# MariBax/self-supervised-depth-estimation

Hardware: AMD Instinct MI355X
Metric: training images/sec at 192x640 bs12 (resnet18 depth+pose, 4-scale photometric+smoothness) (higher is better)
Workload: dtype f32 (1x1 convolutions: bf16x3 split operands, fp32 accumulate); 1 GPU; BASELINE configs[1]: resnet18 depth+pose, 192x640, per-GPU batch 12, 4 scales, frames {0,-1,+1}, automasking, Adam lr 1e-4; random-init weights; global_batch=12, parallelism=dp1, tiebreak_noise=on-device counter RNG, setup_steps=0, step_launch=eager (one launch per kernel)

## Files before the change

include/depthcore.h:

```cpp
#ifndef DEPTHCORE_H
#define DEPTHCORE_H

#include <stddef.h>
#include <stdint.h>

#ifdef __cplusplus
extern "C" {
#endif

#define DC_OK 0
#define DC_EINVAL (-1)
#define DC_ELAUNCH (-2)
#define DC_EWORKSPACE (-3)
#define DC_EEMPTY (-4)

#define DC_MAX_SCALES 4

#define DC_OPT_NO_AUTOMASK 1u
#define DC_OPT_AVG_REPROJ 2u
#define DC_OPT_NO_SSIM 4u
#define DC_OPT_ALIGN_CORNERS 8u
#define DC_OPT_PRED_MASK 32u
#define DC_OPT_PHOTO_SPLIT 64u
#define DC_OPT_PHOTO_FULL 128u
// ... 150 lines not shown
int dc_bn_stats(const float* x, float* part, int N, int C, int HW, int groups, void* stream);
int dc_bn_finalize(const float* part, int nparts, int ppg, double count, const float* gamma, const float* beta,
                   float* running_mean, float* running_var, float* mean, float* invstd, float* scale, float* shift,
                   int C, int groups, float eps, float momentum, void* stream);
int dc_bn_apply(const float* x, const float* res, const float* scale, const float* shift, float* y, void* relu_mask,
                int N, int C, int HW, int relu, int groups, void* stream);
int dc_bn_bwd_finalize(const float* part, int nparts, int ppg, double count, const float* gamma, const float* mean,
                       const float* invstd, float* coef, float* dgamma, float* dbeta, int C, int groups, void* stream);
int dc_bn_bwd_apply(const float* x, const float* gp, const float* coef, float* dx, int N, int C, int HW, int groups,
                    void* stream);

int dc_bn_eval_coef(const float* gamma, const float* beta, const float* running_mean, const float* running_var, float* scale,
                    float* shift, float* invstd, int C, float eps, void* stream);
size_t dc_bn_eval_bwd_workspace(int N, int C, int HW);
int dc_bn_eval_bwd(const float* x, const float* y, const float* gy, const float* scale, const float* running_mean,
                   const float* invstd, float* dx, float* dres, float* dgamma, float* dbeta, void* ws, int N, int C, int HW,
                   int relu, void* stream);

int dc_maxpool3x3s2_fwd(const float* x, float* y, uint8_t* code, int NC, int H, int W, void* stream);
int dc_maxpool3x3s2_bwd(const float* gy, const uint8_t* code, float* dx, int NC, int H, int W, void* stream);
int dc_maxpool3x3s2_bwd_add(const float* gy, const uint8_t* code, float* dx, const float* addend, int NC, int H, int W,
                            void* stream);

size_t dc_wino3x3_workspace(int B, int Ci, int Co, int H, int W);
int dc_wino3x3_fwd(const float* x, const float* weight, float* y, void* ws, int B, int Ci, int Co, int H, int W,
                   void* stream);
int dc_wino3x3_dgrad(const float* gy, const float* weight, float* gx, void* ws, int B, int Ci, int Co, int H, int W,
                     void* stream);
int dc_wino3x3_dgrad_add(const float* gy, const float* weight, float* gx, const float* addend, void* ws, int B, int Ci, int Co,
                         int H, int W, void* stream);

int dc_wino3x3_bn_ok(int B, int Ci, int Co, int H, int W, int groups);
int dc_wino3x3_stat_parts(int B, int Ci, int Co, int H, int W, int groups, int* ppg);
int dc_wino3x3_bwd_parts(int B, int Ci, int Co, int H, int W, int groups, int* ppg);
int dc_wino3x3_fwd_bn(const float* x, const float* weight, float* y, void* ws, int B, int Ci, int Co, int H, int W,
                      const dc_bn_fold* bn, void* stream);
int dc_wino3x3_dgrad_bn(const float* gy, const float* weight, float* gx, const float* addend, void* ws, int B, int Ci, int Co,
                        int H, int W, const dc_bn_fold* bn, void* stream);
int dc_wino3x3_wgrad_bn(const float* x, const float* gy, float* dweight, void* ws, int B, int Ci, int Co, int H, int W,
                        const dc_bn_fold* bn, void* stream);

int dc_conv_profile_enable(int max_launches, int every);
int dc_conv_profile_collect(int kind, double* ms, double* algorithmic_flops, double* executed_flops,
                            double* algorithmic_bytes, int* launches);

size_t dc_wino3x3_wgrad_workspace(int B, int Ci, int Co, int H, int W);
// ... 175 lines not shown
```

self-supervised-depth-estimation_amd/csrc/bn.hip:

```cpp
#include "dc_common.h"

namespace dc {

constexpr int BN_CHUNK = 4096;

__device__ __forceinline__ float block_sum256(float v, float* sm) {
    v = wave_sum(v);
    __syncthreads();
    if ((threadIdx.x & 63) == 0) sm[threadIdx.x >> 6] = v;
    __syncthreads();
    return (sm[0] + sm[1]) + (sm[2] + sm[3]);
}

constexpr int BN_U = 4;
struct BnItems {
    int wave, lane, ipp, nitems, lo, hi, ns, HW;
    __device__ __forceinline__ BnItems(int ns_, int HW_, int lo_, int hi_) : lo(lo_), hi(hi_), ns(ns_), HW(HW_) {
        wave = __builtin_amdgcn_readfirstlane(threadIdx.x >> 6); lane = threadIdx.x & 63;
        if (ns > 1) { ipp = (HW + 255) >> 8; nitems = ((ns - wave + 3) >> 2) * ipp; }
        else { ipp = 1; nitems = (hi - lo + 1023) >> 10; }
    }
    __device__ __forceinline__ bool at(int k, int& nn, int& i) const {
        bool ok;
        if (ns > 1) {
// ... 128 lines not shown
        const size_t base = ((size_t)n * C + c) * HW;
        for (int i = lo + threadIdx.x; i < hi; i += 256) {
            float v = fmaf(x[base + i], a, b);
            if (res) v += res[base + i];
            y[base + i] = relu ? fmaxf(v, 0.f) : v;
        }
    }
}

__device__ __forceinline__ float4 bn_apply_bits(float4 g, unsigned bits) {
    g.x = (bits & 1u) ? g.x : 0.f; g.y = (bits & 2u) ? g.y : 0.f; g.z = (bits & 4u) ? g.z : 0.f; g.w = (bits & 8u) ? g.w : 0.f;
    return g;
}
struct BnMaskWords { unsigned long long w[4]; };
__device__ __forceinline__ unsigned bn_bits_of(const BnMaskWords& m) {
    const int l = threadIdx.x & 63;
    return (unsigned)((m.w[0] >> l) & 1ull) | ((unsigned)((m.w[1] >> l) & 1ull) << 1) | ((unsigned)((m.w[2] >> l) & 1ull) << 2) |
           ((unsigned)((m.w[3] >> l) & 1ull) << 3);
}
__device__ __forceinline__ unsigned bn_bits_of(float4 yv) {
    return (yv.x > 0.f ? 1u : 0u) | (yv.y > 0.f ? 2u : 0u) | (yv.z > 0.f ? 4u : 0u) | (yv.w > 0.f ? 8u : 0u);
}

template <int MODE>
__global__ __launch_bounds__(256) void bn_bwd_stats_kernel(const float* __restrict__ x, const float* __restrict__ y, const float* __restrict__ gy,
                                                           const float* __restrict__ mean, const float* __restrict__ invstd, float* __restrict__ part, int C,
                                                           int HW, int n_per_group, const unsigned long long* __restrict__ mask, int ns) {
    __shared__ float sm[8];
    const int c = blockIdx.y, n0 = blockIdx.z * ns;
    const int gc = (n0 / n_per_group) * C + c;
    const float m = mean[gc], is = invstd[gc];
    const int lo = blockIdx.x * BN_CHUNK, hi = min(lo + BN_CHUNK, HW);
    float s = 0.f, q = 0.f;
    if ((HW & 3) == 0) {
        const BnItems it(ns, HW, lo, hi);
        for (int k0 = 0; k0 < it.nitems; k0 += BN_U) {
            float4 xv[BN_U], g[BN_U], yv[BN_U];
            BnMaskWords mw[BN_U];
            bool ok[BN_U];
#pragma unroll
            for (int u = 0; u < BN_U; ++u) {
                int nn, i;
                ok[u] = it.at(k0 + u, nn, i);
                const size_t plane = (size_t)(n0 + nn) * C + c, off = plane * HW + i;
                xv[u] = *reinterpret_cast<const float4*>(x + off);
                g[u] = *reinterpret_cast<const float4*>(gy + off);
                if (MODE == 1) mw[u] = *reinterpret_cast<const BnMaskWords*>(mask + (plane * ((HW + 255) >> 8) + (i >> 8)) * 4);
                if (MODE == 2) yv[u] = *reinterpret_cast<const float4*>(y + off);
            }
#pragma unroll
            for (int u = 0; u < BN_U; ++u) {
                float4 gg = g[u];
                if (MODE == 1) gg = bn_apply_bits(gg, bn_bits_of(mw[u]));
                if (MODE == 2) gg = bn_apply_bits(gg, bn_bits_of(yv[u]));
                if (!ok[u]) gg = make_float4(0.f, 0.f, 0.f, 0.f);
                s += (gg.x + gg.y) + (gg.z + gg.w);
                q += (gg.x * (xv[u].x - m) + gg.y * (xv[u].y - m)) + (gg.z * (xv[u].z - m) + gg.w * (xv[u].w - m));
            }
        }
    } else {
        const size_t base = ((size_t)n0 * C + c) * HW;
        for (int i = lo + threadIdx.x; i < hi; i += 256) {
            float g = gy[base + i];
            if (MODE != 0 && !(y[base + i] > 0.f)) g = 0.f;
            s += g; q += g * (x[base + i] - m);
        }
    }
    block_sum256x2(s, q, sm);
    q *= is;
    if (threadIdx.x == 0) {
        float* o = part + (((size_t)c * gridDim.z + blockIdx.z) * gridDim.x + blockIdx.x) * 2;
        o[0] = s; o[1] = q;
    }
}

template <int MODE>
__global__ __launch_bounds__(256) void bn_bwd_apply_kernel(const float* __restrict__ x, const float* __restrict__ y, const float* __restrict__ gy,
                                                           const float* __restrict__ mean, const float* __restrict__ invstd, const float* __restrict__ gamma,
                                                           const float* __restrict__ part, float* __restrict__ dgamma, float* __restrict__ dbeta, float* __restrict__ dx,
                                                           float* __restrict__ dres, int C, int HW, int n_per_group,
                                                           int groups, const unsigned long long* __restrict__ mask, int ns) {
    const int c = blockIdx.y, n0 = blockIdx.z * ns, n = n0;
    const int nparts = gridDim.z * gridDim.x, per = nparts / groups;
    const int gidx = n / n_per_group;
    const float count = (float)n_per_group * (float)HW;
    float s, q;
    bn_reduce_partials(part, c, nparts, per, gidx, s, q);
    if (blockIdx.x == 0 && n == 0) {
        float ts = 0.f, tq = 0.f;
        for (int g2 = 0; g2 < groups; ++g2) {
            float s2, q2;
            bn_reduce_partials(part, c, nparts, per, g2, s2, q2);
            ts += s2; tq += q2;
        }
        if (threadIdx.x == 0) {
            if (dbeta) dbeta[c] = ts;
            if (dgamma) dgamma[c] = tq;
        }
    }
    const int gc = gidx * C + c;
    const float m = mean[gc], is = invstd[gc], k = gamma[c] * is, a = s / count, bq = (q / count) * is;
    const int lo = blockIdx.x * BN_CHUNK, hi = min(lo + BN_CHUNK, HW);
    if ((HW & 3) == 0) {
        const BnItems it(ns, HW, lo, hi);
        for (int k0 = 0; k0 < it.nitems; k0 += BN_U) {
            float4 xv[BN_U], g[BN_U], yv[BN_U];
            BnMaskWords mw[BN_U];
            size_t off[BN_U];
            bool ok[BN_U];
#pragma unroll
            for (int u = 0; u < BN_U; ++u) {
                int nn, i;
                ok[u] = it.at(k0 + u, nn, i);
                const size_t plane = (size_t)(n0 + nn) * C + c;
                off[u] = plane * HW + i;
                xv[u] = *reinterpret_cast<const float4*>(x + off[u]);
                g[u] = *reinterpret_cast<const float4*>(gy + off[u]);
                if (MODE == 1) mw[u] = *reinterpret_cast<const BnMaskWords*>(mask + (plane * ((HW + 255) >> 8) + (i >> 8)) * 4);
                if (MODE == 2) yv[u] = *reinterpret_cast<const float4*>(y + off[u]);
            }
#pragma unroll
            for (int u = 0; u < BN_U; ++u) {
                float4 gg = g[u];
                if (MODE == 1) gg = bn_apply_bits(gg, bn_bits_of(mw[u]));
                if (MODE == 2) gg = bn_apply_bits(gg, bn_bits_of(yv[u]));
                float4 d;
                d.x = k * (gg.x - a - (xv[u].x - m) * bq); d.y = k * (gg.y - a - (xv[u].y - m) * bq);
                d.z = k * (gg.z - a - (xv[u].z - m) * bq); d.w = k * (gg.w - a - (xv[u].w - m) * bq);
                if (ok[u]) {
                    if (dres) *reinterpret_cast<float4*>(dres + off[u]) = gg;
                    *reinterpret_cast<float4*>(dx + off[u]) = d;
                }
            }
        }
    } else {
        const size_t base = ((size_t)n * C + c) * HW;
        for (int i = lo + threadIdx.x; i < hi; i += 256) {
            float g = gy[base + i];
            if (MODE != 0 && !(y[base + i] > 0.f)) g = 0.f;
            if (dres) dres[base + i] = g;
            dx[base + i] = k * (g - a - (x[base + i] - m) * bq);
        }
    }
}

}

using namespace dc;
#define ST ((hipStream_t)stream)

static int bn_ns(int n_per_group, int HW) {
    if ((HW & 3) || HW * 2 > BN_CHUNK) return 1;
    int best = 1;
    for (int d = 2; d <= n_per_group; ++d)
        if (n_per_group % d == 0 && d * HW <= BN_CHUNK) best = d;
    return best;
}

extern "C" size_t dc_bn_workspace(int N, int C, int HW) {
    if (N <= 0 || C <= 0 || HW <= 0) return 0;
    return ((size_t)C * N * ceil_div(HW, BN_CHUNK) * 2 + 2 * (size_t)C * N) * sizeof(float);
}
// ... 15 lines not shown
    DC_CHECK_LAUNCH();
    hipLaunchKernelGGL(bn_apply_kernel, dim3(chunks, C, N / ns), dim3(256), 0, ST, x, res, (const float*)part, save_mean,
                       save_invstd, running_mean, running_var, gamma, beta, y, C, HW, relu, N / groups, groups, eps, momentum,
                       (HW & 3) ? (unsigned long long*)nullptr : (unsigned long long*)relu_mask, ns);
    DC_CHECK_LAUNCH();
    return DC_OK;
}

extern "C" int dc_bn_relu_bwd(const float* x, const float* y, const float* gy, const float* gamma,
                              const float* save_mean, const float* save_invstd, float* dx, float* dres, float* dgamma,
                              float* dbeta, void* ws, const void* relu_mask, int N, int C, int HW, int relu, int groups,
                              void* stream) {
    if (!x || !gy || !gamma || !save_mean || !save_invstd || !dx || !ws || N <= 0 || C <= 0 || HW <= 0) return DC_EINVAL;
    const unsigned long long* mk = (HW & 3) ? nullptr : (const unsigned long long*)relu_mask;
    if (relu && !y && !mk) return DC_EINVAL;
    if (groups < 1 || N % groups) return DC_EINVAL;
    const int chunks = ceil_div(HW, BN_CHUNK), ns = bn_ns(N / groups, HW);
    float* part = (float*)ws;
    const dim3 grid(chunks, C, N / ns);
    const int mode = !relu ? 0 : (mk ? 1 : 2);
#define BN_BWD(MODE)                                                                                                             \
    do {                                                                                                                         \
        hipLaunchKernelGGL(bn_bwd_stats_kernel<MODE>, grid, dim3(256), 0, ST, x, y, gy, save_mean, save_invstd, part, C, HW,      \
                           N / groups, mk, ns);                                                                                  \
        DC_CHECK_LAUNCH();                                                                                                       \
        hipLaunchKernelGGL(bn_bwd_apply_kernel<MODE>, grid, dim3(256), 0, ST, x, y, gy, save_mean, save_invstd, gamma,            \
                           (const float*)part, dgamma, dbeta, dx, dres, C, HW, N / groups, groups, mk, ns);                      \
        DC_CHECK_LAUNCH();                                                                                                       \
    } while (0)
    if (mode == 0) BN_BWD(0);
    else if (mode == 1) BN_BWD(1);
    else BN_BWD(2);
#undef BN_BWD
    return DC_OK;
}

namespace dc {

__device__ __forceinline__ void block_sum256x2_all(float& a, float& b, float* sm8) {
    __syncthreads();
    block_sum256x2(a, b, sm8);
}

__global__ __launch_bounds__(256) void bn_finalize_kernel(const float2* __restrict__ part, int nparts, int ppg, float count,
                                                          const float* __restrict__ gamma, const float* __restrict__ beta,
                                                          float* __restrict__ run_mean, float* __restrict__ run_var,
                                                          float* __restrict__ mean, float* __restrict__ invstd,
                                                          float* __restrict__ scale, float* __restrict__ shift, int C, int groups,
                                                          float eps, float momentum) {
    __shared__ float sm[8];
// ... 466 lines not shown
    return dc_maxpool3x3s2_bwd_add(gy, code, dx, nullptr, NC, H, W, stream);
}

extern "C" int dc_maxpool3x3s2_bwd_add(const float* gy, const uint8_t* code, float* dx, const float* addend, int NC, int H, int W,
                                       void* stream) {
    if (!gy || !code || !dx || NC <= 0 || H < 2 || W < 2 || NC > 65535) return DC_EINVAL;
    const int Ho = (H + 2 - 3) / 2 + 1, Wo = (W + 2 - 3) / 2 + 1;
    if (addend && (W & 7)) {
        const int rc = dc_maxpool3x3s2_bwd_add(gy, code, dx, nullptr, NC, H, W, stream);
        return rc != DC_OK ? rc : dc::add_inplace(dx, addend, (size_t)NC * H * W, (hipStream_t)stream);
    }
    if ((W & 7) == 0)
        hipLaunchKernelGGL(dc::maxpool_bwd8_kernel, dim3(dc::ceil_div(H * (W >> 3), 256), NC), dim3(256), 0, (hipStream_t)stream, gy, code,
                           dx, H, W, Ho, Wo, addend);
    else if ((W & 3) == 0)
        hipLaunchKernelGGL(dc::maxpool_bwd_kernel<true>, dim3(dc::ceil_div(H * (W >> 2), 256), NC), dim3(256), 0,
                           (hipStream_t)stream, gy, code, dx, H, W, Ho, Wo);
    else
        hipLaunchKernelGGL(dc::maxpool_bwd_kernel<false>, dim3(dc::ceil_div(H * W, 256), NC), dim3(256), 0,
                           (hipStream_t)stream, gy, code, dx, H, W, Ho, Wo);
    DC_CHECK_LAUNCH();
    return DC_OK;
}
```

self-supervised-depth-estimation_amd/depthcore/_lib.py:

```python
import ctypes
import os
from ctypes import (POINTER, Structure, c_char_p, c_double, c_float, c_int, c_int32, c_size_t, c_uint8, c_uint32,
                    c_uint64, c_void_p)

import torch

_HERE = os.path.dirname(os.path.abspath(__file__))
PRODUCT_LIB = os.path.join(_HERE, "libdepthcore.so")
LIB_PATH = os.environ.get("DEPTHCORE_LIB") or PRODUCT_LIB
IS_VARIANT = os.path.realpath(LIB_PATH) != os.path.realpath(PRODUCT_LIB)
MAX_SCALES = 4

OPT_NO_AUTOMASK = 1
OPT_AVG_REPROJ = 2
OPT_NO_SSIM = 4
OPT_ALIGN_CORNERS = 8
OPT_NO_GRAD = 16
OPT_PRED_MASK = 32
OPT_PHOTO_SPLIT, OPT_PHOTO_FULL = 64, 128
PREC_F32, PREC_BF16 = 0, 1
PASS_FWD, PASS_DGRAD, PASS_WGRAD = 0, 1, 2

_ERR = {-1: "DC_EINVAL (bad shape / null pointer / unsupported option)",
        -2: "DC_ELAUNCH (hip launch failed)",
# ... 113 lines not shown
        "dc_flip_concat": (i, [p, p, i, i, i, i, p]),
        "dc_disp_post_process": (i, [p, p, i, i, i, f, f, p]),
        "dc_depth_png16": (i, [p, p, i, i, i, i, i, f, p]),
        "dc_pose_ate": (i, [p, p, p, i, i, i, p]),
        "dc_disp_render_ws_bytes": (z, [i, i, i, i, i]),
        "dc_disp_render": (i, [p, p, p, p, i, i, i, i, i, c_double, p, z, p]),
        "dc_bn_bwd_finalize": (i, [p, i, i, c_double, p, p, p, p, p, p, i, i, p]),
        "dc_bn_bwd_apply": (i, [p, p, p, p, i, i, i, i, p]),
        "dc_conv1x1_bn_ok": (i, [i, i, i, i, i]),
        "dc_conv1x1_stat_parts": (i, [i, i, i, i, i, i, i, POINTER(c_int)]),
        "dc_conv1x1_bwd_parts": (i, [i, i, i, i, i, i, POINTER(c_int)]),
        "dc_conv1x1_fwd_bn": (i, [p, p, p, i, i, i, i, i, i, POINTER(BnFold), p]),
        "dc_conv1x1_dgrad_bn": (i, [p, p, p, p, i, i, i, i, i, i, POINTER(BnFold), p]),
        "dc_conv1x1_wgrad_bn": (i, [p, p, p, p, i, i, i, i, i, i, POINTER(BnFold), p]),
        "dc_wino3x3_bn_ok": (i, [i, i, i, i, i, i]),
        "dc_wino3x3_stat_parts": (i, [i, i, i, i, i, i, POINTER(c_int)]),
        "dc_wino3x3_bwd_parts": (i, [i, i, i, i, i, i, POINTER(c_int)]),
        "dc_wino3x3_fwd_bn": (i, [p, p, p, p, i, i, i, i, i, POINTER(BnFold), p]),
        "dc_wino3x3_dgrad_bn": (i, [p, p, p, p, p, i, i, i, i, i, POINTER(BnFold), p]),
        "dc_wino3x3_wgrad_bn": (i, [p, p, p, p, i, i, i, i, i, POINTER(BnFold), p]),
        "dc_maxpool3x3s2_fwd": (i, [p, p, p, i, i, i, p]),
        "dc_maxpool3x3s2_bwd": (i, [p, p, p, i, i, i, p]),
        "dc_maxpool3x3s2_bwd_add": (i, [p, p, p, p, i, i, i, p]),
        "dc_conv1x1_dgrad_add2": (i, [p, p, p, p, p, i, i, i, i, i, i, p]),
        "dc_conv3x3_bwd_add": (i, [p, i, i, p, i, p, p, p, p, p, p, p, p, p, p, i, i, i, i, i, i, p]),
        "dc_wino3x3_workspace": (z, [i, i, i, i, i]),
        "dc_wino3x3_fwd": (i, [p, p, p, p, i, i, i, i, i, p]),
        "dc_wino3x3_dgrad": (i, [p, p, p, p, i, i, i, i, i, p]),
        "dc_wino3x3_dgrad_add": (i, [p, p, p, p, p, i, i, i, i, i, p]),
        "dc_conv1x1_fwd": (i, [p, p, p, i, i, i, i, i, i, p]),
        "dc_conv1x1_bias_act_fwd": (i, [p, p, p, p, i, i, i, i, i, i, i, p]),
        "dc_bias_act_bwd": (i, [p, p, p, p, i, i, i, i, p]),
        "dc_conv1x1_dgrad": (i, [p, p, p, i, i, i, i, i, i, p]),
        "dc_conv1x1_dgrad_add": (i, [p, p, p, p, i, i, i, i, i, i, p]),
        "dc_conv1x1_wgrad_workspace": (z, [i, i, i, i, i, i]),
        "dc_conv1x1_wgrad": (i, [p, p, p, p, i, i, i, i, i, i, p]),
        "dc_conv_profile_enable": (i, [i, i]),
        "dc_conv_profile_collect": (i, [i, p, p, p, p, p]),
        "dc_wino3x3_wgrad_workspace": (z, [i, i, i, i, i]),
        "dc_wino3x3_wgrad": (i, [p, p, p, p, i, i, i, i, i, p]),
        "dc_stem_supported": (i, [i, i, i, i, i]),
        "dc_stem_fwd": (i, [p, i, f, f, p, p, p, i, i, i, i, p]),
        "dc_stem_wgrad": (i, [p, i, f, f, p, p, p, i, i, i, i, p]),
        "dc_adam_chunk": (i, []),
        "dc_adam_step": (i, [p, p, p, p, i, f, c_double, c_double, f, p]),
        "dc_convs2_supported": (i, [i, i, i, i, i, i]),
# ... 129 lines not shown
```

self-supervised-depth-estimation_amd/depthcore/ops.py:

```python
import collections
import contextlib
import ctypes
import os
import threading
import weakref

import torch

from . import _lib
from ._lib import PhotoDesc, check, ptr, stream


DepthcoreError = _lib.DepthcoreError


def _c(t):
    return t if t.is_contiguous() else t.contiguous()


_decision_observers = []


def add_decision_observer(fn):
    _decision_observers.append(fn)
# ... 1039 lines not shown
        ctx.skip = skip if (skip is not None and x.requires_grad) else None
        if ctx.skip is not None:
            ctx.skip.arm()
        return y

    @staticmethod
    def backward(ctx, gy):
        L = _lib.lib()
        (code,) = ctx.saved_tensors
        N, C, H, W = ctx.dims
        g_c = _c(gy)
        dx = torch.empty(N, C, H, W, dtype=torch.float32, device=gy.device)
        add = ctx.skip.take() if ctx.skip is not None else None
        if add is not None and (tuple(add.shape) != (N, C, H, W) or not add.is_contiguous()):
            raise _lib.DepthcoreError("SkipSum: gradient %s does not match the pooled tensor %s" % (tuple(add.shape), (N, C, H, W)))
        check(L.dc_maxpool3x3s2_bwd_add(ptr(g_c), code.data_ptr(), ptr(dx), ptr(add), N * C, H, W, stream(g_c)), "dc_maxpool3x3s2_bwd_add")
        return dx, None


def maxpool3x3s2(x, skip=None):
    return _MaxPool.apply(x, skip)


class _WinoConv(torch.autograd.Function):
    @staticmethod
    def forward(ctx, x, weight, fork=None):
        L = _lib.lib()
        xx, ww = _c(x.detach()), _c(weight.detach())
        B, Ci, H, W = xx.shape
        Co = ww.shape[0]
        y = torch.empty(B, Co, H, W, dtype=torch.float32, device=xx.device)
        ctx.prec = _use_precision(_precision[0])
        ws = torch.empty(L.dc_wino3x3_workspace(B, Ci, Co, H, W), dtype=torch.uint8, device=xx.device)
        check(L.dc_wino3x3_fwd(ptr(xx), ptr(ww), ptr(y), ws.data_ptr(), B, Ci, Co, H, W, stream(xx)), "dc_wino3x3_fwd")
        ctx.save_for_backward(xx, ww)
        ctx.slot = _slot(weight)
        ctx.param = _lane_param(ctx, 1, weight)
        ctx.fork = fork if x.requires_grad else None
        return y

    @staticmethod
    def backward(ctx, gy):
        L = _lib.lib()
        xx, ww = ctx.saved_tensors
        B, Ci, H, W = xx.shape
        Co = ww.shape[0]
# ... 620 lines not shown
```

self-supervised-depth-estimation_amd/networks/resnet_encoder.py:

```python
import os

import numpy as np
import torch
import torch.nn as nn

from depthcore import bnfold as _bnf
from depthcore import ops as _ops


def _bn_act(x, bn, res=None, relu=True, groups=1, fork=None):
    if bn.training:
        return _ops.bn_relu(x, bn, res, relu, groups, fork)
    return _ops.bn_eval(x, bn, res, relu)


CONV_S2 = True
GEMM_1X1 = True
WINO_TRUNK = True
STEM_FUSED = True


BN_FOLD = int(os.environ.get("DC_BN_FOLD", "-1"))


def _fold_level(bottleneck):
    return BN_FOLD if BN_FOLD >= 0 else (3 if bottleneck else 0)


GRAD_FORK = True
SKIP_SUMS = os.environ.get("DC_GRAD_SUMS", "1") != "0"


def _fork_for(block, x):
    c = block.conv1
    if not (GRAD_FORK and block.downsample is None and block.training and x.is_cuda and x.requires_grad and x.dtype == torch.float32
            and torch.is_grad_enabled() and c.stride == (1, 1) and c.groups == 1 and c.bias is None and x.numel() * 4 < 0x7fffffff):
        return None
    if c.kernel_size == (3, 3) and WINO_TRUNK and c.padding == (1, 1) and c.dilation == (1, 1) and x.shape[-1] % 2 == 0:
        return _ops.GradFork()
    if c.kernel_size == (1, 1) and GEMM_1X1 and c.padding == (0, 0):
        return _ops.GradFork()
    return None
# ... 234 lines not shown


class ResnetEncoder(nn.Module):

    def __init__(self, num_layers, pretrained, num_input_images=1):
        super().__init__()
        if num_layers not in _CFG:
            raise ValueError("{} is not a valid number of resnet layers".format(num_layers))
        if pretrained is True:
            raise RuntimeError("pretrained=True downloads the ImageNet weights (networks/resnet_encoder.py:53); pass the "
                               "torchvision state dict or the path of its .pth file as `pretrained` instead")
        self.num_ch_enc = np.array([64, 64, 128, 256, 512])
        self.encoder = ResNetTrunk(num_layers, num_input_images)
        if pretrained:
            load_imagenet_weights(self.encoder, pretrained, num_input_images)
        if num_layers > 34:
            self.num_ch_enc[1:] *= 4
        self._nbt = None

    def _apply(self, fn, *a, **k):
        self._nbt = None
        return super()._apply(fn, *a, **k)

    def forward_pairs(self, f_prev, f_cur, f_next):
        frames = (f_prev, f_cur, f_next)
        if STEM_FUSED and _ops.stem_supported(frames, self.encoder.conv1.weight):
            return self._trunk(_ops.stem_conv(frames, self.encoder.conv1.weight), 2)
        pairs = torch.cat([torch.cat([f_prev, f_cur], 1), torch.cat([f_cur, f_next], 1)], 0)
        return self.forward(pairs, bn_groups=2)

    def forward_pair(self, f_a, f_b):
        frames = (f_a, f_b)
        if STEM_FUSED and _ops.stem_supported(frames, self.encoder.conv1.weight):
            return self._trunk(_ops.stem_conv(frames, self.encoder.conv1.weight), 1)
        return self.forward(torch.cat([f_a, f_b], 1))

    def forward(self, input_image, bn_groups=1):
        e = self.encoder
        if STEM_FUSED and input_image.shape[1] == 3 and _ops.stem_supported((input_image,), e.conv1.weight):
            return self._trunk(_ops.stem_conv((input_image,), e.conv1.weight), bn_groups)
        x = (input_image - 0.45) / 0.225
        return self._trunk(_conv(e.conv1, x), bn_groups)

    def _trunk(self, x, bn_groups):
        e = self.encoder
        e._g[0] = int(bn_groups)
        self.features = []
        x = _bn_act(x, e.bn1, groups=e._g[0])
        tag = SKIP_SUMS and self.training and x.is_cuda and x.requires_grad and torch.is_grad_enabled()

        def feature(t):
            if tag:
                t._dc_skip = _ops.SkipSum()
            self.features.append(t)
            return t
        feature(x)
        feature(e.layer1(_ops.maxpool3x3s2(x, _ops.skip_of(x)) if x.is_cuda else e.maxpool(x)))
        feature(e.layer2(self.features[-1]))
        feature(e.layer3(self.features[-1]))
        self.features.append(e.layer4(self.features[-1]))
        if self.training:
            if self._nbt is None:
                self._nbt = [m.num_batches_tracked for m in e.modules() if isinstance(m, nn.BatchNorm2d)]
            torch._foreach_add_(self._nbt, int(bn_groups))
        e._g[0] = 1
        return self.features
```

self-supervised-depth-estimation_amd/trainer.py:

```python
import contextlib
import json
import os
import types

import numpy as np
import torch
import torch.nn.functional as F
import torch.optim as optim

import networks
from layers import (BackprojectDepth, Project3D, SSIM, disp_to_depth, get_smooth_loss, grid_sample,
                    interpolate_bilinear, transformation_from_parameters)
from depthcore import ops
from depthcore.ops import WinoWeightCache
from depthcore.ddp import GradBuckets, agree_all, broadcast_parameters


def default_options(**kw):
    from options import MonodepthOptions
    o = MonodepthOptions().parse([])
    o.weights_init = "scratch"
    for k, v in kw.items():
        setattr(o, k, v)
    return o
# ... 245 lines not shown
        else:
            features = self.models["encoder"](inputs[("color_aug", 0, 0)])
            outputs = dict(self.models["depth"](features))
        if self.opt.predictive_mask:
            outputs["predictive_mask"] = self.models["predictive_mask"](features)
        return outputs

    def _depth_branch_shared(self, inputs):
        ids = list(self.opt.frame_ids)
        B = self.opt.batch_size
        all_features = self.models["encoder"](torch.cat([inputs[("color_aug", i, 0)] for i in ids], 0))
        features = {k: [f[i * B:(i + 1) * B] for f in all_features] for i, k in enumerate(ids)}
        outputs = dict(self.models["depth"](features[0]))
        if self.opt.predictive_mask:
            outputs["predictive_mask"] = self.models["predictive_mask"](features[0])
        return outputs, features

    def predict_poses(self, inputs, features):
        if self.opt.pose_model_type != "separate_resnet" or self.opt.pose_model_input != "pairs":
            return self._predict_poses_modes(inputs, features)
        outputs = {}
        pose_feats = {f: inputs[("color_aug", f, 0)] for f in (-1, 0, 1)}
        B = pose_feats[0].shape[0]
        feats = self.models["pose_encoder"].forward_pairs(pose_feats[-1], pose_feats[0], pose_feats[1])
        axisangle, translation, Ts = self.models["pose"].forward_poses([feats], [(0, B, 0, 1), (B, B, 0, 0)])
        for i, f in enumerate((-1, 1)):
            outputs[("axisangle", 0, f)] = axisangle[i * B:(i + 1) * B]
            outputs[("translation", 0, f)] = translation[i * B:(i + 1) * B]
            outputs[("cam_T_cam", 0, f)] = Ts[i]
        return outputs

    def _poses(self, pose, pose_inputs, groups):
        if self.opt.pose_model_type != "posecnn":
            return pose.forward_poses(pose_inputs, groups)
        axisangle, translation = pose(pose_inputs)
        Ts = [transformation_from_parameters(axisangle[r0:r0 + rows, slot], translation[r0:r0 + rows, slot], invert=bool(inv))
              for r0, rows, slot, inv in groups]
        return axisangle, translation, Ts

    def _predict_poses_modes(self, inputs, features):
        o, outputs = self.opt, {}
        pose = self.models["pose"]
        if self.num_pose_frames == 2:
            feats = {f: features[f] for f in o.frame_ids} if o.pose_model_type == "shared" else \
                {f: inputs[("color_aug", f, 0)] for f in (-1, 0, 1)}
            for f in (-1, 1):
                pose_inputs = [feats[f], feats[0]] if f < 0 else [feats[0], feats[f]]
# ... 436 lines not shown
```

Measured before the change: 1112 images/s.

## Fuse stem BatchNorm, ReLU and 3x3 maxpool in forward and backward

```diff
diff --git a/include/depthcore.h b/include/depthcore.h
--- a/include/depthcore.h
+++ b/include/depthcore.h
@@ -196,6 +196,14 @@
 int dc_maxpool3x3s2_bwd_add(const float* gy, const uint8_t* code, float* dx, const float* addend, int NC, int H, int W,
                             void* stream);
 
+int dc_bn_relu_pool_supported(int N, int C, int H, int W);
+int dc_bn_relu_pool_fwd(const float* x, const float* gamma, const float* beta, float* y, float* pooled, uint8_t* code,
+                        float* save_mean, float* save_invstd, float* save_ab, float* running_mean, float* running_var,
+                        void* ws, int N, int C, int H, int W, float eps, float momentum, int groups, void* stream);
+int dc_bn_relu_pool_bwd(const float* x, const float* gpooled, const uint8_t* code, const float* addend, const float* gy,
+                        const float* gamma, const float* save_mean, const float* save_invstd, const float* save_ab, float* dx, float* dgamma,
+                        float* dbeta, void* ws, int N, int C, int H, int W, int groups, void* stream);
+
 size_t dc_wino3x3_workspace(int B, int Ci, int Co, int H, int W);
 int dc_wino3x3_fwd(const float* x, const float* weight, float* y, void* ws, int B, int Ci, int Co, int H, int W,
                    void* stream);
diff --git a/self-supervised-depth-estimation_amd/csrc/bn.hip b/self-supervised-depth-estimation_amd/csrc/bn.hip
--- a/self-supervised-depth-estimation_amd/csrc/bn.hip
+++ b/self-supervised-depth-estimation_amd/csrc/bn.hip
@@ -174,14 +174,69 @@
     return (yv.x > 0.f ? 1u : 0u) | (yv.y > 0.f ? 2u : 0u) | (yv.z > 0.f ? 4u : 0u) | (yv.w > 0.f ? 8u : 0u);
 }
 
+struct BnPoolSrc {
+    const uint8_t* code;
+    const float* addend;
+    const float* ab;
+    const float* post;
+    int W, Ho, Wo;
+};
+struct BnPoolItem {
+    float4 add, post;
+    float2 g01[2];
+    float g2[2];
+    unsigned c01[2], c2[2];
+    int yy, x0, oy[2];
+    bool has3;
+};
+__device__ __forceinline__ void bn_pool_load(BnPoolItem& t, const BnPoolSrc& ps, const float* __restrict__ gp, size_t plane, int HW, int i) {
+    t.yy = i / ps.W; t.x0 = i - t.yy * ps.W;
+    t.oy[0] = t.yy >> 1; t.oy[1] = min((t.yy + 1) >> 1, ps.Ho - 1);
+    const int oxb = t.x0 >> 1;
+    t.has3 = oxb + 2 < ps.Wo;
+    if (ps.addend) t.add = *reinterpret_cast<const float4*>(ps.addend + plane * HW + i);
+    if (ps.post) t.post = *reinterpret_cast<const float4*>(ps.post + plane * HW + i);
+#pragma unroll
+    for (int r = 0; r < 2; ++r) {
+        const size_t o = (plane * ps.Ho + t.oy[r]) * ps.Wo + oxb;
+        t.c01[r] = *reinterpret_cast<const unsigned short*>(ps.code + o);
+        t.g01[r] = *reinterpret_cast<const float2*>(gp + o);
+        t.c2[r] = ps.code[o + (t.has3 ? 2 : 0)];
+        t.g2[r] = gp[o + (t.has3 ? 2 : 0)];
+    }
+}
+__device__ __forceinline__ float4 bn_pool_gather(const BnPoolItem& t, const BnPoolSrc& ps) {
+    float4 out = ps.addend ? t.add : make_float4(0.f, 0.f, 0.f, 0.f);
+#pragma unroll
+    for (int r = 0; r < 2; ++r) {
+        const int k3 = (r == 1 && t.oy[1] == t.oy[0]) ? 300 : (t.yy - (t.oy[r] * 2 - 1)) * 3;
+        const int c0 = (int)(t.c01[r] & 255u), c1 = (int)(t.c01[r] >> 8), c2 = t.has3 ? (int)t.c2[r] : 255;
+        const float g0 = t.g01[r].x, g1 = t.g01[r].y, g2 = t.g2[r];
+        out.x = c0 == k3 + 1 ? out.x + g0 : out.x;
+        out.y = c0 == k3 + 2 ? out.y + g0 : out.y;
+        out.y = c1 == k3 ? out.y + g1 : out.y;
+        out.z = c1 == k3 + 1 ? out.z + g1 : out.z;
+        out.w = c1 == k3 + 2 ? out.w + g1 : out.w;
+        out.w = c2 == k3 ? out.w + g2 : out.w;
+    }
+    if (ps.post) { out.x += t.post.x; out.y += t.post.y; out.z += t.post.z; out.w += t.post.w; }
+    return out;
+}
+__device__ __forceinline__ unsigned bn_bits_of(float4 xv, float a, float b) {
+    return (fmaf(xv.x, a, b) > 0.f ? 1u : 0u) | (fmaf(xv.y, a, b) > 0.f ? 2u : 0u) | (fmaf(xv.z, a, b) > 0.f ? 4u : 0u) |
+           (fmaf(xv.w, a, b) > 0.f ? 8u : 0u);
+}
+
 template <int MODE>
 __global__ __launch_bounds__(256) void bn_bwd_stats_kernel(const float* __restrict__ x, const float* __restrict__ y, const float* __restrict__ gy,
                                                            const float* __restrict__ mean, const float* __restrict__ invstd, float* __restrict__ part, int C,
-                                                           int HW, int n_per_group, const unsigned long long* __restrict__ mask, int ns) {
+                                                           int HW, int n_per_group, const unsigned long long* __restrict__ mask, int ns, BnPoolSrc ps) {
     __shared__ float sm[8];
     const int c = blockIdx.y, n0 = blockIdx.z * ns;
     const int gc = (n0 / n_per_group) * C + c;
     const float m = mean[gc], is = invstd[gc];
+    float pa = 0.f, pb = 0.f;
+    if (MODE == 3) { pa = ps.ab[2 * gc]; pb = ps.ab[2 * gc + 1]; }
     const int lo = blockIdx.x * BN_CHUNK, hi = min(lo + BN_CHUNK, HW);
     float s = 0.f, q = 0.f;
     if ((HW & 3) == 0) {
@@ -189,6 +244,7 @@
         for (int k0 = 0; k0 < it.nitems; k0 += BN_U) {
             float4 xv[BN_U], g[BN_U], yv[BN_U];
             BnMaskWords mw[BN_U];
+            BnPoolItem pi[BN_U];
             bool ok[BN_U];
 #pragma unroll
             for (int u = 0; u < BN_U; ++u) {
@@ -196,17 +252,23 @@
                 ok[u] = it.at(k0 + u, nn, i);
                 const size_t plane = (size_t)(n0 + nn) * C + c, off = plane * HW + i;
                 xv[u] = *reinterpret_cast<const float4*>(x + off);
-                g[u] = *reinterpret_cast<const float4*>(gy + off);
+                if (MODE == 3) bn_pool_load(pi[u], ps, gy, plane, HW, i);
+                else g[u] = *reinterpret_cast<const float4*>(gy + off);
                 if (MODE == 1) mw[u] = *reinterpret_cast<const BnMaskWords*>(mask + (plane * ((HW + 255) >> 8) + (i >> 8)) * 4);
                 if (MODE == 2) yv[u] = *reinterpret_cast<const float4*>(y + off);
             }
 #pragma unroll
             for (int u = 0; u < BN_U; ++u) {
-                float4 gg = g[u];
+                float4 gg = MODE == 3 ? bn_pool_gather(pi[u], ps) : g[u];
                 if (MODE == 1) gg = bn_apply_bits(gg, bn_bits_of(mw[u]));
                 if (MODE == 2) gg = bn_apply_bits(gg, bn_bits_of(yv[u]));
+                if (MODE == 3) gg = bn_apply_bits(gg, bn_bits_of(xv[u], pa, pb));
                 if (!ok[u]) gg = make_float4(0.f, 0.f, 0.f, 0.f);
                 s += (gg.x + gg.y) + (gg.z + gg.w);
+                if (MODE == 3) {
+                    q += fmaf(gg.x, xv[u].x - m, __fmul_rn(gg.y, xv[u].y - m)) + fmaf(gg.z, xv[u].z - m, __fmul_rn(gg.w, xv[u].w - m));
+                    continue;
+                }
                 q += (gg.x * (xv[u].x - m) + gg.y * (xv[u].y - m)) + (gg.z * (xv[u].z - m) + gg.w * (xv[u].w - m));
             }
         }
@@ -214,7 +276,7 @@
         const size_t base = ((size_t)n0 * C + c) * HW;
         for (int i = lo + threadIdx.x; i < hi; i += 256) {
             float g = gy[base + i];
-            if (MODE != 0 && !(y[base + i] > 0.f)) g = 0.f;
+            if ((MODE == 1 || MODE == 2) && !(y[base + i] > 0.f)) g = 0.f;
             s += g; q += g * (x[base + i] - m);
         }
     }
@@ -231,7 +293,7 @@
                                                            const float* __restrict__ mean, const float* __restrict__ invstd, const float* __restrict__ gamma,
                                                            const float* __restrict__ part, float* __restrict__ dgamma, float* __restrict__ dbeta, float* __restrict__ dx,
                                                            float* __restrict__ dres, int C, int HW, int n_per_group,
-                                                           int groups, const unsigned long long* __restrict__ mask, int ns) {
+                                                           int groups, const unsigned long long* __restrict__ mask, int ns, BnPoolSrc ps) {
     const int c = blockIdx.y, n0 = blockIdx.z * ns, n = n0;
     const int nparts = gridDim.z * gridDim.x, per = nparts / groups;
     const int gidx = n / n_per_group;
@@ -252,12 +314,15 @@
     }
     const int gc = gidx * C + c;
     const float m = mean[gc], is = invstd[gc], k = gamma[c] * is, a = s / count, bq = (q / count) * is;
+    float pa = 0.f, pb = 0.f;
+    if (MODE == 3) { pa = ps.ab[2 * gc]; pb = ps.ab[2 * gc + 1]; }
     const int lo = blockIdx.x * BN_CHUNK, hi = min(lo + BN_CHUNK, HW);
     if ((HW & 3) == 0) {
         const BnItems it(ns, HW, lo, hi);
         for (int k0 = 0; k0 < it.nitems; k0 += BN_U) {
             float4 xv[BN_U], g[BN_U], yv[BN_U];
             BnMaskWords mw[BN_U];
+            BnPoolItem pi[BN_U];
             size_t off[BN_U];
             bool ok[BN_U];
 #pragma unroll
@@ -267,15 +332,17 @@
                 const size_t plane = (size_t)(n0 + nn) * C + c;
                 off[u] = plane * HW + i;
                 xv[u] = *reinterpret_cast<const float4*>(x + off[u]);
-                g[u] = *reinterpret_cast<const float4*>(gy + off[u]);
+                if (MODE == 3) bn_pool_load(pi[u], ps, gy, plane, HW, i);
+                else g[u] = *reinterpret_cast<const float4*>(gy + off[u]);
                 if (MODE == 1) mw[u] = *reinterpret_cast<const BnMaskWords*>(mask + (plane * ((HW + 255) >> 8) + (i >> 8)) * 4);
                 if (MODE == 2) yv[u] = *reinterpret_cast<const float4*>(y + off[u]);
             }
 #pragma unroll
             for (int u = 0; u < BN_U; ++u) {
-                float4 gg = g[u];
+                float4 gg = MODE == 3 ? bn_pool_gather(pi[u], ps) : g[u];
                 if (MODE == 1) gg = bn_apply_bits(gg, bn_bits_of(mw[u]));
                 if (MODE == 2) gg = bn_apply_bits(gg, bn_bits_of(yv[u]));
+                if (MODE == 3) gg = bn_apply_bits(gg, bn_bits_of(xv[u], pa, pb));
                 float4 d;
                 d.x = k * (gg.x - a - (xv[u].x - m) * bq); d.y = k * (gg.y - a - (xv[u].y - m) * bq);
                 d.z = k * (gg.z - a - (xv[u].z - m) * bq); d.w = k * (gg.w - a - (xv[u].w - m) * bq);
@@ -289,7 +356,7 @@
         const size_t base = ((size_t)n * C + c) * HW;
         for (int i = lo + threadIdx.x; i < hi; i += 256) {
             float g = gy[base + i];
-            if (MODE != 0 && !(y[base + i] > 0.f)) g = 0.f;
+            if ((MODE == 1 || MODE == 2) && !(y[base + i] > 0.f)) g = 0.f;
             if (dres) dres[base + i] = g;
             dx[base + i] = k * (g - a - (x[base + i] - m) * bq);
         }
@@ -351,10 +418,10 @@
 #define BN_BWD(MODE)                                                                                                             \
     do {                                                                                                                         \
         hipLaunchKernelGGL(bn_bwd_stats_kernel<MODE>, grid, dim3(256), 0, ST, x, y, gy, save_mean, save_invstd, part, C, HW,      \
-                           N / groups, mk, ns);                                                                                  \
+                           N / groups, mk, ns, BnPoolSrc{});                                                                     \
         DC_CHECK_LAUNCH();                                                                                                       \
         hipLaunchKernelGGL(bn_bwd_apply_kernel<MODE>, grid, dim3(256), 0, ST, x, y, gy, save_mean, save_invstd, gamma,            \
-                           (const float*)part, dgamma, dbeta, dx, dres, C, HW, N / groups, groups, mk, ns);                      \
+                           (const float*)part, dgamma, dbeta, dx, dres, C, HW, N / groups, groups, mk, ns, BnPoolSrc{});         \
         DC_CHECK_LAUNCH();                                                                                                       \
     } while (0)
     if (mode == 0) BN_BWD(0);
@@ -867,3 +934,145 @@
     DC_CHECK_LAUNCH();
     return DC_OK;
 }
+
+namespace dc {
+
+constexpr int POOL_IT = 2;
+template <bool WRITE_Y>
+__global__ __launch_bounds__(256) void bn_relu_pool_fwd_kernel(const float* __restrict__ x, const float* __restrict__ part, float* mean,
+                                                               float* invstd, float* ab, float* run_mean, float* run_var,
+                                                               const float* __restrict__ gamma, const float* __restrict__ beta,
+                                                               float* __restrict__ y, float* __restrict__ pooled, uint8_t* __restrict__ code,
+                                                               int C, int H, int W, int Ho, int Wo, int n_per_group, int groups,
+                                                               int nparts, float eps, float momentum) {
+    const size_t plane = blockIdx.y;
+    const int n = blockIdx.y / C, c = blockIdx.y - n * C;
+    const int Wo2 = Wo >> 1;
+    const float* p = x + plane * H * W;
+    float4 f[POOL_IT][3];
+    float e[POOL_IT][3];
+    int oy[POOL_IT], ox0[POOL_IT];
+    bool live[POOL_IT];
+#pragma unroll
+    for (int t = 0; t < POOL_IT; ++t) {
+        const int i = (blockIdx.x * POOL_IT + t) * 256 + threadIdx.x;
+        live[t] = i < Ho * Wo2;
+        const int il = live[t] ? i : 0;
+        oy[t] = il / Wo2; ox0[t] = (il - oy[t] * Wo2) * 2;
+#pragma unroll
+        for (int ky = 0; ky < 3; ++ky) {
+            const int yy = min(max(oy[t] * 2 - 1 + ky, 0), H - 1);
+            const float* row = p + (size_t)yy * W + 2 * ox0[t];
+            f[t][ky] = *reinterpret_cast<const float4*>(row);
+            e[t][ky] = row[ox0[t] > 0 ? -1 : 0];
+        }
+    }
+    const int per = nparts / groups;
+    const int gidx = n / n_per_group;
+    const float count = (float)n_per_group * (float)(H * W);
+    float s, q;
+    bn_reduce_partials(part, c, nparts, per, gidx, s, q);
+    const float m = s / count;
+    const float var = fmaxf(q / count - m * m, 0.f);
+    const float is = rsqrtf(var + eps);
+    const float a = is * gamma[c], b = beta[c] - m * a;
+    if (blockIdx.x == 0 && threadIdx.x == 0 && n == gidx * n_per_group) {
+        mean[gidx * C + c] = m; invstd[gidx * C + c] = is;
+        ab[(gidx * C + c) * 2] = a; ab[(gidx * C + c) * 2 + 1] = b;
+    }
+    if (blockIdx.x == 0 && n == 0 && run_mean) {
+        float rm = run_mean[c], rv = run_var[c];
+        for (int g2 = 0; g2 < groups; ++g2) {
+            float s2, q2;
+            bn_reduce_partials(part, c, nparts, per, g2, s2, q2);
+            const float m2 = s2 / count, v2 = fmaxf(q2 / count - m2 * m2, 0.f);
+            rm = (1.f - momentum) * rm + momentum * m2;
+            rv = (1.f - momentum) * rv + momentum * v2 * (count / fmaxf(count - 1.f, 1.f));
+        }
+        if (threadIdx.x == 0) { run_mean[c] = rm; run_var[c] = rv; }
+    }
+#pragma unroll
+    for (int t = 0; t < POOL_IT; ++t) {
+        if (!live[t]) continue;
+#pragma unroll
+        for (int ky = 0; ky < 3; ++ky) {
+            f[t][ky].x = fmaxf(fmaf(f[t][ky].x, a, b), 0.f); f[t][ky].y = fmaxf(fmaf(f[t][ky].y, a, b), 0.f);
+            f[t][ky].z = fmaxf(fmaf(f[t][ky].z, a, b), 0.f); f[t][ky].w = fmaxf(fmaf(f[t][ky].w, a, b), 0.f);
+            e[t][ky] = fmaxf(fmaf(e[t][ky], a, b), 0.f);
+        }
+        if (WRITE_Y) {
+            float* yp = y + plane * H * W + 2 * ox0[t];
+            *reinterpret_cast<float4*>(yp + (size_t)(oy[t] * 2) * W) = f[t][1];
+            if (oy[t] * 2 + 1 < H) *reinterpret_cast<float4*>(yp + (size_t)(oy[t] * 2 + 1) * W) = f[t][2];
+        }
+        float ba = -INFINITY, bb = -INFINITY;
+        int ca = 0, cb = 0;
+#pragma unroll
+        for (int ky = 0; ky < 3; ++ky) {
+            const int yy = oy[t] * 2 - 1 + ky;
+            if (yy < 0 || yy >= H) continue;
+            const float4 v = f[t][ky];
+            const float ev = e[t][ky];
+            if (ox0[t] > 0) { if (ev > ba || ev != ev) { ba = ev; ca = ky * 3; } }
+            if (v.x > ba || v.x != v.x) { ba = v.x; ca = ky * 3 + 1; }
+            if (v.y > ba || v.y != v.y) { ba = v.y; ca = ky * 3 + 2; }
+            if (v.y > bb || v.y != v.y) { bb = v.y; cb = ky * 3; }
+            if (v.z > bb || v.z != v.z) { bb = v.z; cb = ky * 3 + 1; }
+            if (v.w > bb || v.w != v.w) { bb = v.w; cb = ky * 3 + 2; }
+        }
+        const size_t o = plane * Ho * Wo + (size_t)oy[t] * Wo + ox0[t];
+        *reinterpret_cast<float2*>(pooled + o) = make_float2(ba, bb);
+        *reinterpret_cast<uchar2*>(code + o) = make_uchar2((uint8_t)ca, (uint8_t)cb);
+    }
+}
+
+}
+
+extern "C" int dc_bn_relu_pool_supported(int N, int C, int H, int W) {
+    if (N <= 0 || C <= 0 || H < 2 || W < 8 || (W & 7)) return 0;
+    if ((long long)N * C > 65535 || (long long)H * W > 0x7fffffffLL / 4) return 0;
+    return 1;
+}
+
+extern "C" int dc_bn_relu_pool_fwd(const float* x, const float* gamma, const float* beta, float* y, float* pooled, uint8_t* code,
+                                   float* save_mean, float* save_invstd, float* save_ab, float* running_mean, float* running_var,
+                                   void* ws, int N, int C, int H, int W, float eps, float momentum, int groups, void* stream) {
+    if (!x || !gamma || !beta || !pooled || !code || !save_mean || !save_invstd || !save_ab || !ws) return DC_EINVAL;
+    if (!dc_bn_relu_pool_supported(N, C, H, W) || groups < 1 || N % groups) return DC_EINVAL;
+    const int HW = H * W, Ho = (H - 1) / 2 + 1, Wo = W / 2;
+    const int chunks = ceil_div(HW, BN_CHUNK), ns = bn_ns(N / groups, HW);
+    float* part = (float*)ws;
+    hipLaunchKernelGGL(bn_stats_kernel, dim3(chunks, C, N / ns), dim3(256), 0, ST, x, part, C, HW, ns);
+    DC_CHECK_LAUNCH();
+    const dim3 grid(ceil_div(Ho * (Wo >> 1), 256 * POOL_IT), N * C);
+    if (y)
+        hipLaunchKernelGGL(bn_relu_pool_fwd_kernel<true>, grid, dim3(256), 0, ST, x, (const float*)part, save_mean, save_invstd, save_ab,
+                           running_mean, running_var, gamma, beta, y, pooled, code, C, H, W, Ho, Wo, N / groups, groups,
+                           (N / ns) * chunks, eps, momentum);
+    else
+        hipLaunchKernelGGL(bn_relu_pool_fwd_kernel<false>, grid, dim3(256), 0, ST, x, (const float*)part, save_mean, save_invstd, save_ab,
+                           running_mean, running_var, gamma, beta, y, pooled, code, C, H, W, Ho, Wo, N / groups, groups,
+                           (N / ns) * chunks, eps, momentum);
+    DC_CHECK_LAUNCH();
+    return DC_OK;
+}
+
+extern "C" int dc_bn_relu_pool_bwd(const float* x, const float* gpooled, const uint8_t* code, const float* addend, const float* gy,
+                                   const float* gamma, const float* save_mean, const float* save_invstd, const float* save_ab, float* dx, float* dgamma,
+                                   float* dbeta, void* ws, int N, int C, int H, int W, int groups, void* stream) {
+    if (!x || !gpooled || !code || !gamma || !save_mean || !save_invstd || !save_ab || !dx || !ws) return DC_EINVAL;
+    if (!dc_bn_relu_pool_supported(N, C, H, W) || groups < 1 || N % groups) return DC_EINVAL;
+    const int HW = H * W, Ho = (H - 1) / 2 + 1, Wo = W / 2;
+    const int chunks = ceil_div(HW, BN_CHUNK), ns = bn_ns(N / groups, HW);
+    float* part = (float*)ws;
+    const dim3 grid(chunks, C, N / ns);
+    const BnPoolSrc ps{code, addend, save_ab, gy, W, Ho, Wo};
+    hipLaunchKernelGGL(bn_bwd_stats_kernel<3>, grid, dim3(256), 0, ST, x, (const float*)nullptr, gpooled, save_mean, save_invstd, part, C,
+                       HW, N / groups, (const unsigned long long*)nullptr, ns, ps);
+    DC_CHECK_LAUNCH();
+    hipLaunchKernelGGL(bn_bwd_apply_kernel<3>, grid, dim3(256), 0, ST, x, (const float*)nullptr, gpooled, save_mean, save_invstd, gamma,
+                       (const float*)part, dgamma, dbeta, dx, (float*)nullptr, C, HW, N / groups, groups,
+                       (const unsigned long long*)nullptr, ns, ps);
+    DC_CHECK_LAUNCH();
+    return DC_OK;
+}
diff --git a/self-supervised-depth-estimation_amd/depthcore/_lib.py b/self-supervised-depth-estimation_amd/depthcore/_lib.py
--- a/self-supervised-depth-estimation_amd/depthcore/_lib.py
+++ b/self-supervised-depth-estimation_amd/depthcore/_lib.py
@@ -159,6 +159,9 @@
         "dc_maxpool3x3s2_fwd": (i, [p, p, p, i, i, i, p]),
         "dc_maxpool3x3s2_bwd": (i, [p, p, p, i, i, i, p]),
         "dc_maxpool3x3s2_bwd_add": (i, [p, p, p, p, i, i, i, p]),
+        "dc_bn_relu_pool_supported": (i, [i, i, i, i]),
+        "dc_bn_relu_pool_fwd": (i, [p, p, p, p, p, p, p, p, p, p, p, p, i, i, i, i, f, f, i, p]),
+        "dc_bn_relu_pool_bwd": (i, [p, p, p, p, p, p, p, p, p, p, p, p, p, i, i, i, i, i, p]),
         "dc_conv1x1_dgrad_add2": (i, [p, p, p, p, p, i, i, i, i, i, i, p]),
         "dc_conv3x3_bwd_add": (i, [p, i, i, p, i, p, p, p, p, p, p, p, p, p, p, i, i, i, i, i, i, p]),
         "dc_wino3x3_workspace": (z, [i, i, i, i, i]),
diff --git a/self-supervised-depth-estimation_amd/depthcore/ops.py b/self-supervised-depth-estimation_amd/depthcore/ops.py
--- a/self-supervised-depth-estimation_amd/depthcore/ops.py
+++ b/self-supervised-depth-estimation_amd/depthcore/ops.py
@@ -1085,6 +1085,77 @@
     return _MaxPool.apply(x, skip)
 
 
+def bn_relu_pool_supported(x):
+    return (x.is_cuda and x.dtype == torch.float32 and x.dim() == 4
+            and bool(_lib.lib().dc_bn_relu_pool_supported(*[int(d) for d in x.shape])))
+
+
+class _BNReLUPool(torch.autograd.Function):
+
+    @staticmethod
+    def forward(ctx, x, gamma, beta, running_mean, running_var, eps, momentum, groups, skip, want_y):
+        L = _lib.lib()
+        xx = _c(x.detach())
+        g, b = _c(gamma.detach()), _c(beta.detach())
+        N, C, H, W = xx.shape
+        Ho, Wo = (H - 1) // 2 + 1, (W - 1) // 2 + 1
+        dev = xx.device
+        y = torch.empty_like(xx) if want_y else None
+        pooled = torch.empty(N, C, Ho, Wo, dtype=torch.float32, device=dev)
+        code = torch.empty(N, C, Ho, Wo, dtype=torch.uint8, device=dev)
+        stats = torch.empty(4, groups * C, dtype=torch.float32, device=dev)
+        mean, invstd, ab = stats[0], stats[1], stats[2:].view(groups * C, 2)
+        ws = torch.empty(L.dc_bn_workspace(N, C, H * W), dtype=torch.uint8, device=dev)
+        check(L.dc_bn_relu_pool_fwd(ptr(xx), ptr(g), ptr(b), ptr(y), ptr(pooled), code.data_ptr(), ptr(mean), ptr(invstd), ptr(ab),
+                                    ptr(running_mean), ptr(running_var), ws.data_ptr(), N, C, H, W, float(eps), float(momentum),
+                                    int(groups), stream(xx)), "dc_bn_relu_pool_fwd")
+        ctx.set_materialize_grads(False)
+        ctx.save_for_backward(xx, g, stats, code)
+        if want_y:
+            _record_kink("relu", y)
+        else:
+            def form_y():
+                yy, sc, sh = torch.empty_like(xx), ab[:, 0].contiguous(), ab[:, 1].contiguous()
+                check(L.dc_bn_apply(ptr(xx), None, ptr(sc), ptr(sh), ptr(yy), None, N, C, H * W, 1, int(groups), stream(xx)), "dc_bn_apply")
+                return yy
+            _record_kink("relu", form_y)
+        _record_kink("maxpool", code)
+        ctx.groups = int(groups)
+        ctx.slots = (_slot(gamma), _slot(beta))
+        ctx.skip = skip if (skip is not None and want_y and any(ctx.needs_input_grad[:3])) else None
+        if ctx.skip is not None:
+            ctx.skip.arm()
+        if y is None:
+            return None, pooled
+        return y, pooled
+
+    @staticmethod
+    def backward(ctx, gy, gpooled):
+        L = _lib.lib()
+        xx, g, stats, code = ctx.saved_tensors
+        mean, invstd, ab = stats[0], stats[1], stats[2:].view(-1, 2)
+        groups = ctx.groups
+        N, C, H, W = xx.shape
+        add = ctx.skip.take() if ctx.skip is not None else None
+        if add is not None and (tuple(add.shape) != (N, C, H, W) or not add.is_contiguous()):
+            raise _lib.DepthcoreError("SkipSum: gradient %s does not match the pooled tensor %s" % (tuple(add.shape), (N, C, H, W)))
+        dx = torch.empty_like(xx)
+        dgamma = _grad_dst(ctx.slots[0], g)
+        dbeta = _grad_dst(ctx.slots[1], g)
+        ws = torch.empty(L.dc_bn_workspace(N, C, H * W), dtype=torch.uint8, device=xx.device)
+        if gpooled is None:
+            gpooled = torch.zeros(N, C, code.shape[2], code.shape[3], dtype=torch.float32, device=xx.device)
+        check(L.dc_bn_relu_pool_bwd(ptr(xx), ptr(_c(gpooled)), code.data_ptr(), ptr(add), ptr(_c(gy)) if gy is not None else None,
+                                    ptr(g), ptr(mean), ptr(invstd), ptr(ab), ptr(dx), ptr(dgamma), ptr(dbeta), ws.data_ptr(),
+                                    N, C, H, W, groups, stream(xx)), "dc_bn_relu_pool_bwd")
+        return dx, dgamma, dbeta, None, None, None, None, None, None, None
+
+
+def bn_relu_pool(x, bn, groups=1, skip=None, want_y=True):
+    mom = 0.1 if bn.momentum is None else bn.momentum
+    return _BNReLUPool.apply(x, bn.weight, bn.bias, bn.running_mean, bn.running_var, bn.eps, mom, groups, skip, want_y)
+
+
 class _WinoConv(torch.autograd.Function):
     @staticmethod
     def forward(ctx, x, weight, fork=None):
diff --git a/self-supervised-depth-estimation_amd/networks/resnet_encoder.py b/self-supervised-depth-estimation_amd/networks/resnet_encoder.py
--- a/self-supervised-depth-estimation_amd/networks/resnet_encoder.py
+++ b/self-supervised-depth-estimation_amd/networks/resnet_encoder.py
@@ -18,6 +18,7 @@
 GEMM_1X1 = True
 WINO_TRUNK = True
 STEM_FUSED = True
+STEM_POOL_FUSED = os.environ.get("DC_STEM_POOL", "1") != "0"
 
 
 BN_FOLD = int(os.environ.get("DC_BN_FOLD", "-1"))
@@ -298,40 +299,53 @@
         self._nbt = None
         return super()._apply(fn, *a, **k)
 
-    def forward_pairs(self, f_prev, f_cur, f_next):
+    def forward_pairs(self, f_prev, f_cur, f_next, features="all"):
         frames = (f_prev, f_cur, f_next)
         if STEM_FUSED and _ops.stem_supported(frames, self.encoder.conv1.weight):
-            return self._trunk(_ops.stem_conv(frames, self.encoder.conv1.weight), 2)
+            return self._trunk(_ops.stem_conv(frames, self.encoder.conv1.weight), 2, features)
         pairs = torch.cat([torch.cat([f_prev, f_cur], 1), torch.cat([f_cur, f_next], 1)], 0)
-        return self.forward(pairs, bn_groups=2)
-
-    def forward_pair(self, f_a, f_b):
+        return self.forward(pairs, bn_groups=2, features=features)
+
+    def forward_pair(self, f_a, f_b, features="all"):
         frames = (f_a, f_b)
         if STEM_FUSED and _ops.stem_supported(frames, self.encoder.conv1.weight):
-            return self._trunk(_ops.stem_conv(frames, self.encoder.conv1.weight), 1)
-        return self.forward(torch.cat([f_a, f_b], 1))
-
-    def forward(self, input_image, bn_groups=1):
+            return self._trunk(_ops.stem_conv(frames, self.encoder.conv1.weight), 1, features)
+        return self.forward(torch.cat([f_a, f_b], 1), features=features)
+
+    def forward(self, input_image, bn_groups=1, features="all"):
         e = self.encoder
         if STEM_FUSED and input_image.shape[1] == 3 and _ops.stem_supported((input_image,), e.conv1.weight):
-            return self._trunk(_ops.stem_conv((input_image,), e.conv1.weight), bn_groups)
+            return self._trunk(_ops.stem_conv((input_image,), e.conv1.weight), bn_groups, features)
         x = (input_image - 0.45) / 0.225
-        return self._trunk(_conv(e.conv1, x), bn_groups)
-
-    def _trunk(self, x, bn_groups):
+        return self._trunk(_conv(e.conv1, x), bn_groups, features)
+
+    def _trunk(self, x, bn_groups, features="all"):
+        if features not in ("all", "last"):
+            raise ValueError("features must be 'all' or 'last', got %r" % (features,))
         e = self.encoder
         e._g[0] = int(bn_groups)
         self.features = []
-        x = _bn_act(x, e.bn1, groups=e._g[0])
-        tag = SKIP_SUMS and self.training and x.is_cuda and x.requires_grad and torch.is_grad_enabled()
-
-        def feature(t):
-            if tag:
-                t._dc_skip = _ops.SkipSum()
+
+        def tagged(t):
+            return SKIP_SUMS and self.training and t.is_cuda and t.requires_grad and torch.is_grad_enabled()
+
+        def feature(t, skip=None):
+            if t is not None and tag:
+                t._dc_skip = skip if skip is not None else _ops.SkipSum()
             self.features.append(t)
             return t
-        feature(x)
-        feature(e.layer1(_ops.maxpool3x3s2(x, _ops.skip_of(x)) if x.is_cuda else e.maxpool(x)))
+        if STEM_POOL_FUSED and e.bn1.training and x.shape[0] % e._g[0] == 0 and _ops.bn_relu_pool_supported(x):
+            skip = _ops.SkipSum()
+            y, pooled = _ops.bn_relu_pool(x, e.bn1, e._g[0], skip, want_y=features == "all")
+            tag = tagged(pooled)
+            feature(y, skip)
+        else:
+            x = _bn_act(x, e.bn1, groups=e._g[0])
+            tag = tagged(x)
+            pooled = _ops.maxpool3x3s2(x, _ops.skip_of(feature(x))) if x.is_cuda else e.maxpool(feature(x))
+            if features == "last":
+                self.features[0] = None
+        feature(e.layer1(pooled))
         feature(e.layer2(self.features[-1]))
         feature(e.layer3(self.features[-1]))
         self.features.append(e.layer4(self.features[-1]))
diff --git a/self-supervised-depth-estimation_amd/trainer.py b/self-supervised-depth-estimation_amd/trainer.py
--- a/self-supervised-depth-estimation_amd/trainer.py
+++ b/self-supervised-depth-estimation_amd/trainer.py
@@ -291,7 +291,7 @@
         outputs = {}
         pose_feats = {f: inputs[("color_aug", f, 0)] for f in (-1, 0, 1)}
         B = pose_feats[0].shape[0]
-        feats = self.models["pose_encoder"].forward_pairs(pose_feats[-1], pose_feats[0], pose_feats[1])
+        feats = self.models["pose_encoder"].forward_pairs(pose_feats[-1], pose_feats[0], pose_feats[1], features="last")
         axisangle, translation, Ts = self.models["pose"].forward_poses([feats], [(0, B, 0, 1), (B, B, 0, 0)])
         for i, f in enumerate((-1, 1)):
             outputs[("axisangle", 0, f)] = axisangle[i * B:(i + 1) * B]
```

Result: no change. 1130 images/s, median of 6 (+1.6%).
